# akankshabaranwal/graph-algorithm-image-segmentation-GPGPU

Hardware: NVIDIA B200
Metric: Mpixel/s end-to-end segmentation (1080p, Boruvka-Felzenszwalb, 4-connected) (higher is better)
Workload: dtype f32+u64

## Files before the change

graph-algorithm-image-segmentation-gpgpu_b200/__init__.py:

```python
import ctypes as C
import os
import subprocess

import numpy as np

_HERE = os.path.dirname(os.path.abspath(__file__))
_ROOT = os.path.dirname(_HERE)
CSRC = os.path.join(_HERE, "csrc")
LIB_PATH = os.environ.get("GSEG_LIB") or os.path.join(_HERE, "libgseg.so")
CLI_PATH = os.path.join(_HERE, "gseg")
BATCH_PATH = os.path.join(_HERE, "gseg_batch")
HEADER = os.path.join(_ROOT, "include", "gseg.h")

FELZ, HIER, SUPERPIX = 0, 1, 2
MEM_HOST, MEM_DEVICE = 0, 1
FLAG_HOST_LOOP = 1
FLAG_NO_DEDUP = 2
CAP_SUPERPIX, CAP_WIDE_SIGMA, CAP_LEVELS, CAP_JPEG = 1, 2, 4, 8
JPEG_AUTO, JPEG_OWN, JPEG_NVJPEG = 0, 1, 2
OUT_NONE, OUT_LABELS, OUT_HIERARCHY = 0, 1, 2
POOL_MAXLEVELS = 64

NVCC_FLAGS = ["-gencode", "arch=compute_100a,code=sm_100a", "-O3", "-lineinfo", "-std=c++17",
              "-Xcompiler", "-fPIC,-ffp-contract=off"]
# ... 88 lines not shown
    L.gseg_segment_jpeg_async.argtypes = [vp, vp, C.c_size_t, C.POINTER(Params), C.POINTER(i32), C.POINTER(i32)]
    L.gseg_input_rgb.argtypes = [vp, vp, i32]
    L.gseg_jpeg_decode_async.argtypes = [vp, vp, C.c_size_t, vp, C.c_size_t, vp, C.POINTER(i32), C.POINTER(i32)]
    L.gseg_set_jpeg_backend.argtypes = [vp, i32]
    L.gseg_jpeg_backend_used.argtypes = [vp]
    L.gseg_num_levels.argtypes = [vp]
    L.gseg_num_components.argtypes = [vp, i32]
    L.gseg_labels.argtypes = [vp, i32, vp, i32]
    L.gseg_labels_async.argtypes = [vp, i32, vp, i32]
    L.gseg_sync.argtypes = [vp]
    L.gseg_labels_all.argtypes = [vp, vp, i32, i32]
    L.gseg_colorize.argtypes = [vp, i32, u64, vp, i32]
    L.gseg_weights.argtypes = [vp, vp, i32]
    L.gseg_blurred.argtypes = [vp, vp, i32]
    L.gseg_stats.argtypes = [vp, C.POINTER(RoundStat), i32]
    i64 = C.c_int64
    L.gseg_export_graph.argtypes = [vp, i32, C.POINTER(i64), C.POINTER(i64), vp, vp, vp, vp, vp, i64, i64]
    L.gseg_blurred_rows.argtypes = [vp, i32, i32, vp, i32]
    L.gseg_segment_graph.argtypes = [vp, i64, vp, vp, i64, vp, vp, vp, C.POINTER(Params), vp]
    L.gseg_synth.argtypes = [vp, vp, i32, i32, u64, i32]
    L.gseg_synth_rows.argtypes = [vp, vp, i32, i32, i32, u64, i32]
    L.gseg_set_profiling.argtypes = [vp, i32]
    L.gseg_profile_read.argtypes = [vp, C.POINTER(KernelTime), i32]
    L.gseg_launch_count.argtypes = [vp]
    L.gseg_launch_count.restype = C.c_longlong
    L.gseg_sort_pairs_u64.argtypes = [vp, vp, vp, C.c_int64, i32, i32]
    L.gseg_reserve.argtypes = [vp, C.c_uint32]
    L.gseg_set_dedup.argtypes = [vp, i32, C.c_uint32, C.c_uint32, C.c_uint32]
    L.gseg_host_alloc.argtypes = [C.c_size_t]
    L.gseg_host_alloc.restype = vp
# ... 295 lines not shown
        Int = np.ascontiguousarray(Int, np.float32)
        ea = np.ascontiguousarray(ea, np.uint32)
        eb = np.ascontiguousarray(eb, np.uint32)
        w = np.ascontiguousarray(w, np.float32)
        out = np.empty(len(size), np.int32)
        n = self._ck(self.L.gseg_segment_graph(self.h, len(size), size.ctypes.data, Int.ctypes.data, len(ea),
                                               ea.ctypes.data, eb.ctypes.data, w.ctypes.data, C.byref(p),
                                               out.ctypes.data), "gseg_segment_graph")
        return out, n

    def stats(self):
        arr = (RoundStat * 64)()
        n = self._ck(self.L.gseg_stats(self.h, arr, 64), "gseg_stats")
        return [(arr[i].n_components, arr[i].n_edges, arr[i].n_merged, arr[i].phase) for i in range(n)]

    def dedup_rounds(self):
        arr = (RoundStat * 64)()
        n = self._ck(self.L.gseg_stats(self.h, arr, 64), "gseg_stats")
        return [(i, arr[i].n_edges, arr[i].n_edges_dedup) for i in range(n) if arr[i].n_edges_dedup]

    def timeline(self):
        arr = (RoundStat * 64)()
        n = self._ck(self.L.gseg_stats(self.h, arr, 64), "gseg_stats")
        return [(i, arr[i].in_tail, arr[i].us_end, arr[i].us_S, arr[i].us_R, arr[i].us_E, arr[i].n_pages) for i in range(n)]

    def set_profiling(self, on):
        self._ck(self.L.gseg_set_profiling(self.h, int(on)), "gseg_set_profiling")

    def profile(self):
        arr = (KernelTime * 1024)()
# ... 29 lines not shown
```

graph-algorithm-image-segmentation-gpgpu_b200/csrc/gseg_api.cu:

```cuda
#include <cuda_runtime.h>
#include <dlfcn.h>
#include <nvjpeg.h>
#include <limits.h>
#include <stddef.h>
#include <math.h>
#include <stdio.h>
#include <stdlib.h>
#include <string.h>

#include <new>
#include <vector>

#include "../../include/gseg.h"
#include "gseg_kernels.cuh"
#include "gseg_sort.cuh"
#include "gseg_dedup.cuh"
#include "gseg_jpeg.hpp"
#include "gseg_jpeg.cuh"

#define GSEG_MAXMARK 1024
#define GRID_CAP (148 * 8)

struct GsegHead {
    GsegRunParams p;
    RoundState st;
    u32 Vnext, error, ticketC, ticketE, doneE, Eacc[GSEG_MAXR + 1];
    u32 map_skip[GSEG_MAXR + 1], resume_phase;
    u32 stDedupIn[GSEG_MAXR + 1], stDedupOut[GSEG_MAXR + 1];
};
static_assert(offsetof(GsegCtl, Eacc) == offsetof(GsegHead, Eacc), "GsegHead must mirror the head of GsegCtl");
static_assert(offsetof(GsegCtl, resume_phase) == offsetof(GsegHead, resume_phase), "GsegHead must mirror the head of GsegCtl");
static_assert(offsetof(GsegCtl, stDedupOut) == offsetof(GsegHead, stDedupOut), "GsegHead must mirror the head of GsegCtl");
#define GSEG_EPOCHS_PER_RUN (2u * GSEG_MAXR + 8u + 32u)

#define R0_STAGE_MAX_PPW 128

static const size_t TAIL_SMEM = (2 * (size_t)GSEG_TAIL_STAGE + 2 * (NTT / 32)) * sizeof(u32);

struct gseg_ctx {
    int device, max_w, max_h;
    size_t Vmax;
    int Dmax;
    cudaStream_t stream, own_stream;
    uint8_t *d_rgb;
    float *d_tmp, *d_planes, *d_G, *d_wgrid;
    u32 *d_wsel, *d_succ, *d_rank;
    u64 *d_best[2];
    uint2 *d_attr[2];
    long long *d_csum[2];
    float4 *d_cmean[2];
    uint2 *d_eab[2];
    u32 *d_ew[2], *d_pcnt[2], *d_poff[2], *d_pscan;
    u32 *d_arena;
    size_t arena_cap;
    u64 *d_statusC, *d_statusE;
    size_t ntilesC, ntilesE;
    int *d_labels[2];
    GsegCtl *d_ctl, *h_ctl;
    GsegHead *h_head;
    int num_sms, occ_mult;
    u32 filter_shift;
    u32 r0_stage_ppw;
    int tail_cluster;
    bool tail_cluster_env;
    u32 tail_E, tail_V, tail_P;
    u32 run_tail_E, run_tail_V;
    int nbig_hint;
    int hint_w, hint_h, hint_variant, hint_conn;
    SortScratch sort;
    DedupDev *d_dd;
    u64 *d_winner;
    size_t dd_cap;
    u32 dd_min_edges, dd_min_ratio, dd_V;
    bool dd_on;
    bool dd_skip;
    u64 *d_xkeys;
    u32 *d_xvals, *d_xkeep, *d_xw, *x_w;
// ... 188 lines not shown
        cudaFuncSetAttribute(k_tail<false>, cudaFuncAttributeMaxDynamicSharedMemorySize, (int)TAIL_SMEM);
        if (const char *ev = getenv("GSEG_TAIL_CLUSTER")) want = atoi(ev);
        ctx->tail_cluster = fit_tail_cluster(want);
        ctx->tail_cluster_env = getenv("GSEG_TAIL_CLUSTER") != nullptr;
        ctx->tail_E = 256u * 1024u; ctx->tail_V = 64u * 1024u; ctx->tail_P = 4096u;
        if (const char *ev = getenv("GSEG_TAIL_P")) ctx->tail_P = (u32)strtoul(ev, nullptr, 10);
        if (const char *ev = getenv("GSEG_TAIL_E")) ctx->tail_E = (u32)strtoul(ev, nullptr, 10);
        if (const char *ev = getenv("GSEG_TAIL_V")) ctx->tail_V = (u32)strtoul(ev, nullptr, 10);
        ctx->nbig_hint = -1;
        ctx->occ_mult = 4;
        if (const char *ev = getenv("GSEG_OCC_MULT")) ctx->occ_mult = atoi(ev) > 0 ? atoi(ev) : 4;
        ctx->filter_shift = 6;
        if (const char *ev = getenv("GSEG_FILTER_SHIFT")) ctx->filter_shift = (u32)atoi(ev);
        ctx->r0_stage_ppw = R0_STAGE_MAX_PPW;
        if (const char *ev = getenv("GSEG_R0_STAGE_PPW")) ctx->r0_stage_ppw = (u32)strtoul(ev, nullptr, 10);
    }
    if (e != cudaSuccess) {
        fprintf(stderr, "gseg_create: %s\n", cudaGetErrorString(e));
        gseg_destroy(ctx);
        return GSEG_E_CUDA;
    }
    memset(ctx->h_ctl, 0, sizeof(GsegCtl));
    *out = ctx;
    return GSEG_OK;
}


struct NvJpegApi {
    void *lib;
    decltype(&nvjpegCreateSimple) create;
// ... 385 lines not shown
static void launch_r0_edges(gseg_ctx *c, cudaStream_t s, size_t V, const GsegBufs &B) {
    static bool attr[64] = {false};
    if (!attr[c->device & 63]) { cudaFuncSetAttribute(k_r0_edges<D, SP, true>, cudaFuncAttributeMaxDynamicSharedMemorySize, (int)R0_SMEM); attr[c->device & 63] = true; }
    const size_t pages = (size_t)D * ((V + GSEG_PAGE - 1) / GSEG_PAGE);
    const size_t ntiles = (pages + NT / 32 - 1) / (NT / 32);
    const int grid = (int)(ntiles < (size_t)c->num_sms * c->occ_mult ? ntiles : (size_t)c->num_sms * c->occ_mult);
    if (pages <= (size_t)c->r0_stage_ppw * grid * (NT / 32)) {
        mark(c, s, "k_r0_edges", 0);
        k_r0_edges<D, SP, true><<<grid, NT, R0_SMEM, s>>>(c->d_ctl, B);
    } else {
        mark(c, s, "k_r0_edges_rl", 0);
        k_r0_edges<D, SP, false><<<grid, NT, 0, s>>>(c->d_ctl, B);
    }
}

static void enqueue_round0(gseg_ctx *c, cudaStream_t s) {
    const size_t V = (size_t)c->w * c->h;
    const int variant = c->params.variant, D = c->D;
    const bool sp = variant == GSEG_SUPERPIX;
    const GsegBufs B = bufs_of(c);
    const int ntiles = ((c->w + TW - 1) / TW) * ((c->h + TH - 1) / TH);
    const int ntilesG = ((c->w + TW - 1) / TW) * ((c->h + GH - 1) / GH);
    const int R = c->h_head->p.mask_len - 1;
    if (R >= 1 && R <= 8) {
        mark(c, s, "k_blur_tile", 0);
        switch (R) {
        case 1: launch_blur<1>(c, s, ntiles); break;
        case 2: launch_blur<2>(c, s, ntiles); break;
        case 3: launch_blur<3>(c, s, ntiles); break;
        case 4: launch_blur<4>(c, s, ntiles); break;
// ... 33 lines not shown
    const int cap = c->num_sms * c->occ_mult;
    if (Pb > GSEG_PSCAN_INLINE) {
        mark(c, s, "k_page_scan", r);
        k_page_scan<<<grid_for(Pb, 1024, 64), 1024, 0, s>>>(c->d_ctl, B);
    }
    mark(c, s, "k_succ_scan", r);
    if (sp) k_succ_scan<true><<<grid_for(Vb, NT * CPT, cap) + 1, NT, 0, s>>>(c->d_ctl, B);
    else k_succ_scan<false><<<grid_for(Vb, NT * CPT, cap) + 1, NT, 0, s>>>(c->d_ctl, B);
    mark(c, s, "k_relabel", r);
    if (sp) k_relabel<false, true><<<grid_for(Vb, NT, cap), NT, 0, s>>>(c->d_ctl, B);
    else k_relabel<false, false><<<grid_for(Vb, NT, cap), NT, 0, s>>>(c->d_ctl, B);
    if (sp) {
        mark(c, s, "k_means", r);
        k_means<<<grid_for(Vb, NT, cap), NT, 0, s>>>(c->d_ctl, B);
    }
    mark(c, s, "k_edges", r);
    if (sp) k_edges<true><<<grid_for(Pb, NT / 32, cap), NT, 0, s>>>(c->d_ctl, B);
    else k_edges<false><<<grid_for(Pb, NT / 32, cap), NT, 0, s>>>(c->d_ctl, B);
}

static u32 dedup_V(const gseg_ctx *c) {
    const u32 v = c->dd_V > 2u ? c->dd_V : 2u;
    return v < 65536u ? v : 65536u;
}
static bool dedup_enabled(const gseg_ctx *c) {
    return c->dd_on && c->params.variant != GSEG_SUPERPIX && !(c->params.flags & GSEG_FLAG_NO_DEDUP);
}
static bool dedup_enqueue(const gseg_ctx *c) {
    return dedup_enabled(c) &&
           !(c->dd_skip && c->hint_w == c->w && c->hint_h == c->h && c->hint_variant == c->params.variant && c->hint_conn == c->params.connectivity);
}
static void enqueue_dedup(gseg_ctx *c, cudaStream_t s, int round) {
    const GsegBufs B = bufs_of(c);
// ... 242 lines not shown
    hp->max_levels = p->max_levels > 0 ? p->max_levels : INT_MAX;
    hp->arena_cap = (u32)ctx->arena_cap; hp->edge_slots = (u32)edge_slots(ctx);
    hp->epoch_base = ctx->epoch_next;
    hp->mask_len = len;
    hp->filter_shift = ctx->filter_shift;
    hp->tail_E = ctx->run_tail_E = host_loop ? 0u : ctx->tail_E;
    hp->tail_V = ctx->run_tail_V = host_loop ? 0u : ctx->tail_V;
    hp->tail_P = ctx->tail_P;
    hp->no_dedup = dedup_enabled(ctx) ? 0u : 1u; hp->dd_V = dedup_V(ctx);
    ctx->epoch_next += GSEG_EPOCHS_PER_RUN;
    hh->st.V = (u32)((size_t)w * h); hh->st.E = 0; hh->st.round = 0; hh->st.phase = PH_PRED; hh->st.levels = 0; hh->st.map_off = 0; hh->st.P = 0; hh->st.pad = 0;
    hh->Vnext = hh->st.V; hh->error = DERR_NONE; hh->ticketC = 0; hh->ticketE = 0; hh->doneE = 0;
    memset(hh->Eacc, 0, sizeof(hh->Eacc));
    memset(hh->map_skip, 0, sizeof(hh->map_skip)); hh->resume_phase = PH_DONE;
    memset(hh->stDedupIn, 0, sizeof(hh->stDedupIn)); memset(hh->stDedupOut, 0, sizeof(hh->stDedupOut));
    CK(cudaMemcpyAsync(ctx->d_ctl, hh, sizeof(GsegHead), cudaMemcpyHostToDevice, ctx->stream));

    ctx->n_marks = 0;
    enqueue_round0(ctx, ctx->stream);
    CK(cudaGetLastError());
    if (!host_loop) {
        int nbig = ctx->nbig_hint;
        if (nbig < 0 || ctx->hint_w != w || ctx->hint_h != h || ctx->hint_variant != p->variant ||
            ctx->hint_conn != p->connectivity)
            nbig = estimate_nbig(ctx);
        if (nbig > R - 1) nbig = R - 1;
        const size_t V = (size_t)w * h;
        for (int r = 1; r <= nbig; ++r) enqueue_round(ctx, ctx->stream, r, V, (size_t)ctx->D * (V / GSEG_PAGE + 1));
        if (dedup_enqueue(ctx)) enqueue_dedup(ctx, ctx->stream, -1);
        CK(cudaGetLastError());
// ... 377 lines not shown
    hp->epoch_base = ctx->epoch_next;
    hp->filter_shift = ctx->filter_shift;
    const bool host_loop = (p->flags & GSEG_FLAG_HOST_LOOP) != 0;
    hp->tail_E = ctx->run_tail_E = host_loop ? 0u : ctx->tail_E;
    hp->tail_V = ctx->run_tail_V = host_loop ? 0u : ctx->tail_V;
    hp->tail_P = ctx->tail_P;
    hp->no_dedup = dedup_enabled(ctx) ? 0u : 1u; hp->dd_V = dedup_V(ctx);
    ctx->epoch_next += GSEG_EPOCHS_PER_RUN;
    const u32 P = (u32)((E + GSEG_PAGE - 1) / GSEG_PAGE);
    hh->st.V = (u32)V; hh->st.E = (u32)E; hh->st.round = 1; hh->st.phase = PH_PRED; hh->st.levels = 0; hh->st.map_off = 0;
    hh->st.P = P; hh->st.pad = 0;
    hh->Vnext = (u32)V; hh->error = DERR_NONE; hh->ticketC = 0; hh->ticketE = 0; hh->doneE = 0;
    memset(hh->Eacc, 0, sizeof(hh->Eacc));
    memset(hh->map_skip, 0, sizeof(hh->map_skip)); hh->resume_phase = PH_DONE;
    memset(hh->stDedupIn, 0, sizeof(hh->stDedupIn)); memset(hh->stDedupOut, 0, sizeof(hh->stDedupOut));
    CK(cudaMemcpyAsync(ctx->d_ctl, hh, sizeof(GsegHead), cudaMemcpyHostToDevice, s));
    ctx->n_marks = 0;
    const GsegBufs B = bufs_of(ctx);
    if (P) { ++ctx->launches; k_graph_init<<<grid_for(P, NT / 32), NT, 0, s>>>(B, (u32)E, P); }
    CK(cudaGetLastError());
    ctx->nbig_hint = -1;
    int rc;
    if (host_loop) {
        rc = readback(ctx);
        for (int go; !rc && (go = run_continues(ctx)) != 0;) {
            if (go < 0) { rc = go; break; }
            if (dedup_wanted_host(ctx)) {
                enqueue_dedup(ctx, s, (int)ctx->h_ctl->st.round);
                CK(cudaGetLastError());
                if ((rc = readback(ctx)) != 0) break;
// ... 166 lines not shown
        out[i].n_edges = i == 0 ? 0 : (hc->stDedupIn[i] ? hc->stDedupIn[i] : hc->stE[i]);
        out[i].n_merged = hc->stM[i];
        out[i].phase = (int32_t)hc->stP[i];
        const bool tail = hc->stTail[i] != 0;
        out[i].in_tail = tail ? 1 : 0;
        out[i].n_pages = (int32_t)hc->stPages[i];
        out[i].n_edges_dedup = deduped ? (int32_t)(hc->stDedupOut[i] ? hc->stDedupOut[i] : hc->stE[i]) : 0;
        out[i].us_end = (float)((double)(hc->t_end[i] - hc->t_start) * 1e-3);
        out[i].us_S = tail ? (float)((double)(hc->t_S[i] - hc->t_begin[i]) * 1e-3) : 0.f;
        out[i].us_R = tail ? (float)((double)(hc->t_R[i] - hc->t_S[i]) * 1e-3) : 0.f;
        out[i].us_E = tail ? (float)((double)(hc->t_end[i] - hc->t_R[i]) * 1e-3) : 0.f;
    }
    return n;
}

extern "C" int gseg_synth_rows(gseg_ctx *ctx, uint8_t *out, int w, int y_first, int nrows, uint64_t seed, int mem_kind) {
    if (!ctx || !out || w < 1 || nrows < 1 || y_first < 0) return GSEG_E_ARG;
    if (mem_kind != GSEG_MEM_HOST && mem_kind != GSEG_MEM_DEVICE) return GSEG_E_ARG;
    if (mem_kind == GSEG_MEM_HOST && (size_t)w * nrows > ctx->Vmax) return GSEG_E_SIZE;
    if (ctx->pending) return GSEG_E_STATE;
    CK(cudaSetDevice(ctx->device));
    const size_t V = (size_t)w * nrows;
    uint8_t *dst = mem_kind == GSEG_MEM_DEVICE ? out : ctx->d_rgb;
    ++ctx->launches;
    k_synth<<<grid_for(V, NT), NT, 0, ctx->stream>>>(dst, w, nrows, seed, y_first);
    CK(cudaGetLastError());
    if (mem_kind != GSEG_MEM_DEVICE) CK(cudaMemcpyAsync(out, dst, 3 * V, cudaMemcpyDeviceToHost, ctx->stream));
    CK(cudaStreamSynchronize(ctx->stream));
    return GSEG_OK;
}
// ... 33 lines not shown
    const double En = (r + 1 < (int)h->st.round) ? h->stE[r + 1] : h->st.E;
    const bool sp = c->params.variant == GSEG_SUPERPIX;
    const double acc = sp ? 40 : 16;
    double a = 0, s = 0;
    if (!strcmp(name, "k_blur_tile") || !strcmp(name, "k_blur_h")) a = s = 3 * V0 + 12 * V0;
    else if (!strcmp(name, "k_blur_v")) a = s = 12 * V0 + 12 * V0;
    else if (!strcmp(name, "k_sobel")) a = s = 12 * V0 + 4 * V0;
    else if (!strcmp(name, "k_r0_graph")) a = s = (sp ? 16 : 12) * V0 + 4 * E0 + 8 * V0 + (4 + acc) * Vn;
    else if (!strcmp(name, "k_relabel")) {
        const double attr_in = r == 0 ? (sp ? 12 * V : 0) : (sp ? 32 : 8) * V, out = (sp ? 32 : 8) * Vn;
        a = 4 * V + 4 * V + 4 * V + 4 * V + attr_in + 4 * (V - Vn) + out;
        s = 4 * V + 4 * Vn + 4 * V + attr_in + 4 * (V - Vn) + out;
    }
    else if (!strcmp(name, "k_r0_edges") || !strcmp(name, "k_r0_edges_rl")) { a = 4 * E0 + 8 * E0 + 12 * En + 8 * Vn; s = 4 * E0 + 4 * V0 + 12 * En + 8 * Vn; }
    else if (!strcmp(name, "k_succ_scan")) { a = 8 * V + 8 * V + 16 * V + 8 * V + 8 * V + (4 + acc) * Vn; s = 8 * V + 8 * V + 8 * V + 8 * V + (4 + acc) * Vn; }
    else if (!strcmp(name, "k_edges")) { a = 12 * E + 8 * E + 12 * En + 8 * Vn + (sp ? 32 * En : 0); s = 12 * E + 4 * V + 12 * En + 8 * Vn + (sp ? 16 * Vn : 0); }
    else if (!strcmp(name, "k_means")) a = s = 32 * Vn + 16 * Vn;
    else if (!strcmp(name, "k_page_scan")) a = s = 8.0 * h->stPages[r];
    *algo = a; *strict = s;
}

extern "C" int gseg_profile_read(gseg_ctx *ctx, gseg_kernel_time *out, int cap) {
    if (!ctx || !ctx->valid) return GSEG_E_STATE;
    CK(cudaSetDevice(ctx->device));
    CK(cudaStreamSynchronize(ctx->stream));
    int n = 0;
    for (int i = 0; i + 1 < ctx->n_marks && n < cap; ++i) {
        if (!ctx->mark_name[i]) continue;
        float ms = 0.f;
        if (cudaEventElapsedTime(&ms, ctx->ev[i], ctx->ev[i + 1]) != cudaSuccess) { cudaGetLastError(); continue; }
        if (out) {
// ... 10 lines not shown
```

graph-algorithm-image-segmentation-gpgpu_b200/csrc/gseg_device.cuh:

```cuda
#pragma once
#include <cuda_runtime.h>
#include <stdint.h>

typedef unsigned int u32;
typedef unsigned long long u64;

#define GSEG_KEY_NONE 0xFFFFFFFFFFFFFFFFull
#define GSEG_INF_BITS 0x7F800000u
#define GSEG_MAXR 64
#define GSEG_MAXMASK 64
#define GSEG_PAGE 256u

enum { PH_PRED = 0, PH_MINSIZE = 1, PH_DONE = 2 };
enum { DERR_NONE = 0, DERR_SCAN = 1, DERR_ARENA = 2, DERR_CHASE = 3, DERR_JPEG = 4 , DERR_CHECK = 100  };

#ifdef GSEG_CHECKED
#define GSEG_CHK(ctl, cond, site)                                                         \
    do {                                                                                  \
        if (!(cond)) atomicMax(&(const_cast<GsegCtl *>(ctl))->error, (u32)DERR_CHECK + (u32)(site)); \
    } while (0)
#else
#define GSEG_CHK(ctl, cond, site) ((void)0)
#endif

// ... 21 lines not shown
    u32 P;
    u32 pad;
};

struct GsegCtl {
    GsegRunParams p;
    RoundState st;
    u32 Vnext;
    u32 error;
    u32 ticketC, ticketE;
    u32 doneE;
    u32 Eacc[GSEG_MAXR + 1];
    u32 map_skip[GSEG_MAXR + 1];
    u32 resume_phase;
    u32 stDedupIn[GSEG_MAXR + 1], stDedupOut[GSEG_MAXR + 1];
    u32 map_off[GSEG_MAXR + 1];
    u32 stV[GSEG_MAXR], stE[GSEG_MAXR], stM[GSEG_MAXR], stP[GSEG_MAXR], stVafter[GSEG_MAXR];
    u32 stTail[GSEG_MAXR], stPages[GSEG_MAXR];
    u64 t_start, t_end[GSEG_MAXR], t_begin[GSEG_MAXR], t_S[GSEG_MAXR], t_R[GSEG_MAXR];
};

struct GsegBufs {
    float *planes, *G, *wgrid;
    u32 *succ, *rank, *wsel, *arena;
    u64 *best[2];
    uint2 *attr[2];
    long long *csum[2];
    float4 *cmean[2];
    uint2 *eab[2];
    u32 *ew[2];
// ... 240 lines not shown
```

graph-algorithm-image-segmentation-gpgpu_b200/csrc/gseg_kernels.cuh:

```cuda
#pragma once
#include <cooperative_groups.h>

#include "gseg_device.cuh"

namespace cg = cooperative_groups;

#define NT 256
#ifndef GSEG_LB_SUCC
#define GSEG_LB_SUCC 4
#endif
#ifndef GSEG_LB_EDGES
#define GSEG_LB_EDGES 4
#endif
#define NTT 1024
#define CPT 4
#ifndef RUNWIN
#define RUNWIN 4
#endif

#define TW 64
#ifndef TH
#define TH 32
#endif
#define BW (TW + 4)
// ... 873 lines not shown
    const u32 nwarp = blockDim.x >> 5, nw = gridDim.x * nwarp;
    const bool staged = SPREAD && stage != nullptr && st.V <= GSEG_TAIL_STAGE;
    u32 *s_map = stage, *s_bhi = stage + GSEG_TAIL_STAGE;
    if (staged) {
        for (u32 i = threadIdx.x; i < st.V; i += blockDim.x) s_map[i] = __ldcg(map + i);
        if (filter) {
            const u32 *bhi = reinterpret_cast<const u32 *>(B.best[nxt]) + 1;
            for (u32 i = threadIdx.x; i < Vnext; i += blockDim.x) s_bhi[i] = ld_relaxed_u32(bhi + 2 * (size_t)i);
        }
        __syncthreads();
    }
    constexpr int NQ = ROWS / RW;
    const u32 wid = threadIdx.x >> 5, q = SPREAD ? (wid & (NQ - 1)) : 0u, grp = wid / NQ;
    u32 *s_ex = stage + 2 * GSEG_TAIL_STAGE;
    u32 esum = 0, parity = 0;
    for (u32 g = SPREAD ? grp * gridDim.x + blockIdx.x : blockIdx.x * nwarp + wid; g < ngroups; g += SPREAD ? gridDim.x * (nwarp / NQ) : nw) {
        u32 mycnt = 0u, myoff = 0u;
        if ((u32)lane < G && G * g + lane < P) { mycnt = __ldcg(pc + G * g + lane); myoff = __ldcg(po + G * g + lane); }
        const u32 incl = warp_incl_scan(mycnt, lane);
        const u32 excl = incl - mycnt, cnt = __shfl_sync(0xFFFFFFFFu, incl, 31);
        const u32 out_base = G > 1u ? __ldcg(B.pscan + G * g) : __shfl_sync(0xFFFFFFFFu, myoff, 0);
        u32 written = 0;
        for (u32 c0 = 0; c0 < cnt; c0 += GSEG_PAGE) {
            u32 a[RW], b[RW], wv[RW], m[RW];
#pragma unroll
            for (int j = 0; j < RW; ++j) {
                const u32 i = c0 + 32u * (q * RW + j) + lane;
                u32 k = 0u;
                if (G > 1u) {
#pragma unroll
                    for (u32 step = 8u; step; step >>= 1) {
                        const u32 e = __shfl_sync(0xFFFFFFFFu, excl, (int)(k + step));
                        if (k + step < G && e <= i) k += step;
                    }
                }
                const u32 src = __shfl_sync(0xFFFFFFFFu, myoff, (int)k) + (i - __shfl_sync(0xFFFFFFFFu, excl, (int)k));
                uint2 ab = make_uint2(0u, 0u);
                wv[j] = 0u;
                if (i < cnt) {
                    GSEG_CHK(ctl, src < ctl->p.edge_slots, 7);
                    ab = __ldcg(eab + src); wv[j] = __ldcg(ew + src);
                    GSEG_CHK(ctl, ab.x < st.V && ab.y < st.V, 8);
                }
                a[j] = ab.x; b[j] = ab.y;
            }
            u32 sub = 0;
#pragma unroll
            for (int j = 0; j < RW; ++j) {
                bool keep = false;
                if (c0 + 32u * (q * RW + j) + lane < cnt) {
                    if (staged) { a[j] = s_map[a[j]]; b[j] = s_map[b[j]]; }
                    else { a[j] = ld_prev<!SPREAD>(map + a[j]); b[j] = ld_prev<!SPREAD>(map + b[j]); }
                    keep = a[j] != b[j];
                }
                m[j] = __ballot_sync(0xFFFFFFFFu, keep);
                sub += __popc(m[j]);
// ... 47 lines not shown
        if (q == 0u) {
            if (lane == 0) { B.pcnt[nxt][g] = written; B.poff[nxt][g] = out_base; }
            esum += written;
        }
    }
    if (lane == 0 && esum) atomicAdd(&ctl->Eacc[st.round], esum);
}
template <bool SP, bool SPREAD = false>
__device__ __forceinline__ void phase_E(GsegCtl *ctl, const GsegBufs &B, const RoundState &st, u32 Vnext, u32 *stage = nullptr) {
    if (SPREAD) {
        const u32 G = group_size(st), ngroups = (st.P + G - 1u) / G;
        if (ngroups <= 2u * gridDim.x * (blockDim.x >> 5)) phase_E_rows<SP, true, 2>(ctl, B, st, Vnext, stage);
        else phase_E_rows<SP, true, GSEG_PAGE / 32>(ctl, B, st, Vnext, stage);
    } else {
        phase_E_rows<SP, false, GSEG_PAGE / 32>(ctl, B, st, Vnext, stage);
    }
}

__device__ __forceinline__ void phase_M(const GsegBufs &B, int nxt, u32 Vnext) {
    for (u32 n = ((threadIdx.x >> 5) * gridDim.x + blockIdx.x) * 32u + (threadIdx.x & 31u); n < Vnext; n += gridDim.x * blockDim.x)
        B.cmean[nxt][n] = mean_of(B.csum[nxt], B.attr[nxt], n);
}

template <bool R0, bool SP>
__global__ void __launch_bounds__(NT) k_relabel(const GsegCtl *ctl, GsegBufs B) {
    const RoundState st = ctl->st;
    if (st.phase == PH_DONE || in_tail(ctl, st)) return;
    phase_R<NT, R0, SP>(ctl, B, st);
}
__global__ void __launch_bounds__(NT) k_means(const GsegCtl *ctl, GsegBufs B) {
// ... 23 lines not shown
        if (i < P) B.pscan[i] = wpre + inc - v;
        __syncthreads();
    }
}
template <bool SP>
__global__ void __launch_bounds__(NT, GSEG_LB_SUCC) k_succ_scan(GsegCtl *ctl, GsegBufs B) {
    __shared__ u32 sh[66];
    const RoundState st = ctl->st;
    if (st.phase == PH_DONE || in_tail(ctl, st)) return;
    if (blockIdx.x == gridDim.x - 1) {
        if (group_size(st) > 1u && st.P <= GSEG_PSCAN_INLINE) block_scan_pages(B.pcnt[st.round & 1], st.P, B.pscan, sh);
        return;
    }
    phase_S<SP, false>(ctl, B, st, sh);
}
template <bool SP>
__global__ void __launch_bounds__(NT, GSEG_LB_EDGES) k_edges(GsegCtl *ctl, GsegBufs B) {
    const RoundState st = ctl->st;
    if (st.phase == PH_DONE || in_tail(ctl, st)) return;
    phase_E<SP>(ctl, B, st, ctl->Vnext);
    last_block_advance(ctl, st, group_size(st));
}

template <bool SP>
__global__ void __launch_bounds__(NTT, 1) k_tail(GsegCtl *ctl, GsegBufs B) {
    extern __shared__ __align__(16) u32 tail_stage[];
    __shared__ u32 sh[66];
    cg::cluster_group cl = cg::this_cluster();
    const bool writer = blockIdx.x == 0 && threadIdx.x == 0;
    RoundState st = load_state(ctl);
    cl.sync();
    while (st.phase != PH_DONE && in_tail(ctl, st)) {
        if (writer) ctl->t_begin[st.round] = globaltimer_ns();
        const u32 G = group_size(st);
        if (G > 1u && blockIdx.x == gridDim.x - 1) block_scan_pages(B.pcnt[st.round & 1], st.P, B.pscan, sh);
// ... 267 lines not shown
```

include/gseg.h:

```cpp
#ifndef GSEG_H
#define GSEG_H

#include <stddef.h>
#include <stdint.h>

#ifdef __cplusplus
extern "C" {
#endif

#define GSEG_VERSION 200

#define GSEG_FELZ 0
#define GSEG_HIER 1
#define GSEG_SUPERPIX 2

#define GSEG_MEM_HOST 0
#define GSEG_MEM_DEVICE 1

#define GSEG_FLAG_HOST_LOOP 1u

#define GSEG_FLAG_NO_DEDUP 2u

typedef enum gseg_status {
    GSEG_OK = 0,
// ... 108 lines not shown
                      int64_t *n_joined_edges);

#define GSEG_JPEG_AUTO 0
#define GSEG_JPEG_OWN 1
#define GSEG_JPEG_NVJPEG 2
int gseg_jpeg_info(const void *jpeg, size_t nbytes, int *w, int *h);
int gseg_segment_jpeg_async(gseg_ctx *ctx, const void *jpeg, size_t nbytes, const gseg_params *params, int *w, int *h);
int gseg_segment_jpeg(gseg_ctx *ctx, const void *jpeg, size_t nbytes, const gseg_params *params, int *w, int *h);
int gseg_input_rgb(gseg_ctx *ctx, uint8_t *out_rgb, int mem_kind);
int gseg_jpeg_decode_async(gseg_ctx *ctx, const void *jpeg, size_t nbytes, uint8_t *rgb_out_device, size_t out_capacity,
                           void *cuda_stream, int *w, int *h);
int gseg_set_jpeg_backend(gseg_ctx *ctx, int backend);
int gseg_jpeg_backend_used(const gseg_ctx *ctx);

int gseg_stats(const gseg_ctx *ctx, gseg_round_stat *out, int cap);

int gseg_synth(gseg_ctx *ctx, uint8_t *out_rgb, int w, int h, uint64_t seed, int mem_kind);
int gseg_synth_rows(gseg_ctx *ctx, uint8_t *out_rgb, int w, int y_first, int nrows, uint64_t seed, int mem_kind);

typedef struct gseg_kernel_time {
    char name[24];
    int32_t round;
    float ms;
    double algo_bytes;
    double strict_bytes;
} gseg_kernel_time;
int gseg_set_profiling(gseg_ctx *ctx, int on);
int gseg_profile_read(gseg_ctx *ctx, gseg_kernel_time *out, int cap);
long long gseg_launch_count(const gseg_ctx *ctx);
long long gseg_compaction_count(const gseg_ctx *ctx);
// ... 43 lines not shown
```

Measured before the change: 10050.

## Prefetch edge-group metadata and pages in edge compaction; add optional bulk-copy staged variant

In the default edge-compaction path, each warp now loads group count and offset metadata two groups ahead. It also issues L1 prefetches for the upcoming group's edge and weight cache lines, and switches those loads from L2-only to L1-cached. A new staged kernel variant, selected by an environment threshold that defaults to off, double-buffers whole edge groups into shared memory with bulk async copies and mbarriers. It also records per-round group statistics. The goal is to hide global-memory latency on the edge gather, at the cost of extra registers and an extra L1 prefetch instruction stream.

After: 9452 (median of 6 runs). -5.9%, worse.

```diff
diff --git a/graph-algorithm-image-segmentation-gpgpu_b200/__init__.py b/graph-algorithm-image-segmentation-gpgpu_b200/__init__.py
--- a/graph-algorithm-image-segmentation-gpgpu_b200/__init__.py
+++ b/graph-algorithm-image-segmentation-gpgpu_b200/__init__.py
@@ -126,6 +126,7 @@
     L.gseg_weights.argtypes = [vp, vp, i32]
     L.gseg_blurred.argtypes = [vp, vp, i32]
     L.gseg_stats.argtypes = [vp, C.POINTER(RoundStat), i32]
+    L.gseg_edge_groups.argtypes = [vp, C.POINTER(C.c_int32), i32]
     i64 = C.c_int64
     L.gseg_export_graph.argtypes = [vp, i32, C.POINTER(i64), C.POINTER(i64), vp, vp, vp, vp, vp, i64, i64]
     L.gseg_blurred_rows.argtypes = [vp, i32, i32, vp, i32]
@@ -451,6 +452,11 @@
         n = self._ck(self.L.gseg_stats(self.h, arr, 64), "gseg_stats")
         return [(arr[i].n_components, arr[i].n_edges, arr[i].n_merged, arr[i].phase) for i in range(n)]
 
+    def edge_groups(self):
+        arr = (C.c_int32 * (3 * 64))()
+        n = self._ck(self.L.gseg_edge_groups(self.h, arr, 64), "gseg_edge_groups")
+        return [(arr[3 * i], arr[3 * i + 1], arr[3 * i + 2]) for i in range(n)]
+
     def dedup_rounds(self):
         arr = (RoundStat * 64)()
         n = self._ck(self.L.gseg_stats(self.h, arr, 64), "gseg_stats")
diff --git a/graph-algorithm-image-segmentation-gpgpu_b200/csrc/gseg_api.cu b/graph-algorithm-image-segmentation-gpgpu_b200/csrc/gseg_api.cu
--- a/graph-algorithm-image-segmentation-gpgpu_b200/csrc/gseg_api.cu
+++ b/graph-algorithm-image-segmentation-gpgpu_b200/csrc/gseg_api.cu
@@ -27,13 +27,16 @@
     u32 Vnext, error, ticketC, ticketE, doneE, Eacc[GSEG_MAXR + 1];
     u32 map_skip[GSEG_MAXR + 1], resume_phase;
     u32 stDedupIn[GSEG_MAXR + 1], stDedupOut[GSEG_MAXR + 1];
+    u32 stGroups[GSEG_MAXR + 1][3];
 };
 static_assert(offsetof(GsegCtl, Eacc) == offsetof(GsegHead, Eacc), "GsegHead must mirror the head of GsegCtl");
 static_assert(offsetof(GsegCtl, resume_phase) == offsetof(GsegHead, resume_phase), "GsegHead must mirror the head of GsegCtl");
 static_assert(offsetof(GsegCtl, stDedupOut) == offsetof(GsegHead, stDedupOut), "GsegHead must mirror the head of GsegCtl");
+static_assert(offsetof(GsegCtl, stGroups) == offsetof(GsegHead, stGroups), "GsegHead must mirror the head of GsegCtl");
 #define GSEG_EPOCHS_PER_RUN (2u * GSEG_MAXR + 8u + 32u)
 
 #define R0_STAGE_MAX_PPW 128
+#define EDGE_STAGE_MAX_PPW 0
 
 static const size_t TAIL_SMEM = (2 * (size_t)GSEG_TAIL_STAGE + 2 * (NTT / 32)) * sizeof(u32);
 
@@ -61,6 +64,7 @@
     int num_sms, occ_mult;
     u32 filter_shift;
     u32 r0_stage_ppw;
+    u32 edge_stage_ppw;
     int tail_cluster;
     bool tail_cluster_env;
     u32 tail_E, tail_V, tail_P;
@@ -279,6 +283,8 @@
         if (const char *ev = getenv("GSEG_FILTER_SHIFT")) ctx->filter_shift = (u32)atoi(ev);
         ctx->r0_stage_ppw = R0_STAGE_MAX_PPW;
         if (const char *ev = getenv("GSEG_R0_STAGE_PPW")) ctx->r0_stage_ppw = (u32)strtoul(ev, nullptr, 10);
+        ctx->edge_stage_ppw = EDGE_STAGE_MAX_PPW;
+        if (const char *ev = getenv("GSEG_EDGE_STAGE_PPW")) ctx->edge_stage_ppw = (u32)strtoul(ev, nullptr, 10);
     }
     if (e != cudaSuccess) {
         fprintf(stderr, "gseg_create: %s\n", cudaGetErrorString(e));
@@ -694,6 +700,20 @@
     }
 }
 
+template <bool SP>
+static void launch_edges(gseg_ctx *c, cudaStream_t s, int r, size_t Pb, int cap, const GsegBufs &B) {
+    static bool attr[64] = {false};
+    if (!attr[c->device & 63]) { cudaFuncSetAttribute(k_edges<SP, true>, cudaFuncAttributeMaxDynamicSharedMemorySize, (int)E_SMEM); attr[c->device & 63] = true; }
+    const int grid = grid_for(Pb, NT / 32, cap);
+    if (Pb <= (size_t)c->edge_stage_ppw * grid * (NT / 32)) {
+        mark(c, s, "k_edges", r);
+        k_edges<SP, true><<<grid, NT, E_SMEM, s>>>(c->d_ctl, B);
+    } else {
+        mark(c, s, "k_edges_rl", r);
+        k_edges<SP, false><<<grid, NT, 0, s>>>(c->d_ctl, B);
+    }
+}
+
 static void enqueue_round0(gseg_ctx *c, cudaStream_t s) {
     const size_t V = (size_t)c->w * c->h;
     const int variant = c->params.variant, D = c->D;
@@ -757,9 +777,8 @@
         mark(c, s, "k_means", r);
         k_means<<<grid_for(Vb, NT, cap), NT, 0, s>>>(c->d_ctl, B);
     }
-    mark(c, s, "k_edges", r);
-    if (sp) k_edges<true><<<grid_for(Pb, NT / 32, cap), NT, 0, s>>>(c->d_ctl, B);
-    else k_edges<false><<<grid_for(Pb, NT / 32, cap), NT, 0, s>>>(c->d_ctl, B);
+    if (sp) launch_edges<true>(c, s, r, Pb, cap, B);
+    else launch_edges<false>(c, s, r, Pb, cap, B);
 }
 
 static u32 dedup_V(const gseg_ctx *c) {
@@ -1032,6 +1051,7 @@
     memset(hh->Eacc, 0, sizeof(hh->Eacc));
     memset(hh->map_skip, 0, sizeof(hh->map_skip)); hh->resume_phase = PH_DONE;
     memset(hh->stDedupIn, 0, sizeof(hh->stDedupIn)); memset(hh->stDedupOut, 0, sizeof(hh->stDedupOut));
+    memset(hh->stGroups, 0, sizeof(hh->stGroups));
     CK(cudaMemcpyAsync(ctx->d_ctl, hh, sizeof(GsegHead), cudaMemcpyHostToDevice, ctx->stream));
 
     ctx->n_marks = 0;
@@ -1439,6 +1459,7 @@
     memset(hh->Eacc, 0, sizeof(hh->Eacc));
     memset(hh->map_skip, 0, sizeof(hh->map_skip)); hh->resume_phase = PH_DONE;
     memset(hh->stDedupIn, 0, sizeof(hh->stDedupIn)); memset(hh->stDedupOut, 0, sizeof(hh->stDedupOut));
+    memset(hh->stGroups, 0, sizeof(hh->stGroups));
     CK(cudaMemcpyAsync(ctx->d_ctl, hh, sizeof(GsegHead), cudaMemcpyHostToDevice, s));
     ctx->n_marks = 0;
     const GsegBufs B = bufs_of(ctx);
@@ -1635,6 +1656,17 @@
     return n;
 }
 
+extern "C" int gseg_edge_groups(const gseg_ctx *ctx, int32_t *out, int cap) {
+    if (!ctx || !ctx->valid) return GSEG_E_STATE;
+    const GsegCtl *hc = ctx->h_ctl;
+    const int n = (int)hc->st.round;
+    for (int i = 0; i < n && i < cap && out; ++i) {
+        for (int j = 0; j < 3; ++j) out[3 * i + j] = (int32_t)hc->stGroups[i][j];
+        out[3 * i] -= out[3 * i + 1] + out[3 * i + 2];
+    }
+    return n;
+}
+
 extern "C" int gseg_synth_rows(gseg_ctx *ctx, uint8_t *out, int w, int y_first, int nrows, uint64_t seed, int mem_kind) {
     if (!ctx || !out || w < 1 || nrows < 1 || y_first < 0) return GSEG_E_ARG;
     if (mem_kind != GSEG_MEM_HOST && mem_kind != GSEG_MEM_DEVICE) return GSEG_E_ARG;
@@ -1698,7 +1730,7 @@
     }
     else if (!strcmp(name, "k_r0_edges") || !strcmp(name, "k_r0_edges_rl")) { a = 4 * E0 + 8 * E0 + 12 * En + 8 * Vn; s = 4 * E0 + 4 * V0 + 12 * En + 8 * Vn; }
     else if (!strcmp(name, "k_succ_scan")) { a = 8 * V + 8 * V + 16 * V + 8 * V + 8 * V + (4 + acc) * Vn; s = 8 * V + 8 * V + 8 * V + 8 * V + (4 + acc) * Vn; }
-    else if (!strcmp(name, "k_edges")) { a = 12 * E + 8 * E + 12 * En + 8 * Vn + (sp ? 32 * En : 0); s = 12 * E + 4 * V + 12 * En + 8 * Vn + (sp ? 16 * Vn : 0); }
+    else if (!strcmp(name, "k_edges") || !strcmp(name, "k_edges_rl")) { a = 12 * E + 8 * E + 12 * En + 8 * Vn + (sp ? 32 * En : 0); s = 12 * E + 4 * V + 12 * En + 8 * Vn + (sp ? 16 * Vn : 0); }
     else if (!strcmp(name, "k_means")) a = s = 32 * Vn + 16 * Vn;
     else if (!strcmp(name, "k_page_scan")) a = s = 8.0 * h->stPages[r];
     *algo = a; *strict = s;
diff --git a/graph-algorithm-image-segmentation-gpgpu_b200/csrc/gseg_device.cuh b/graph-algorithm-image-segmentation-gpgpu_b200/csrc/gseg_device.cuh
--- a/graph-algorithm-image-segmentation-gpgpu_b200/csrc/gseg_device.cuh
+++ b/graph-algorithm-image-segmentation-gpgpu_b200/csrc/gseg_device.cuh
@@ -59,6 +59,7 @@
     u32 map_skip[GSEG_MAXR + 1];
     u32 resume_phase;
     u32 stDedupIn[GSEG_MAXR + 1], stDedupOut[GSEG_MAXR + 1];
+    u32 stGroups[GSEG_MAXR + 1][3];
     u32 map_off[GSEG_MAXR + 1];
     u32 stV[GSEG_MAXR], stE[GSEG_MAXR], stM[GSEG_MAXR], stP[GSEG_MAXR], stVafter[GSEG_MAXR];
     u32 stTail[GSEG_MAXR], stPages[GSEG_MAXR];
diff --git a/graph-algorithm-image-segmentation-gpgpu_b200/csrc/gseg_kernels.cuh b/graph-algorithm-image-segmentation-gpgpu_b200/csrc/gseg_kernels.cuh
--- a/graph-algorithm-image-segmentation-gpgpu_b200/csrc/gseg_kernels.cuh
+++ b/graph-algorithm-image-segmentation-gpgpu_b200/csrc/gseg_kernels.cuh
@@ -911,12 +911,33 @@
     const u32 wid = threadIdx.x >> 5, q = SPREAD ? (wid & (NQ - 1)) : 0u, grp = wid / NQ;
     u32 *s_ex = stage + 2 * GSEG_TAIL_STAGE;
     u32 esum = 0, parity = 0;
+    auto meta = [&](u32 gg, u32 &cnt, u32 &off) {
+        cnt = 0u; off = 0u;
+        if ((u32)lane < G && G * gg + lane < P) { cnt = __ldcg(pc + G * gg + lane); off = __ldcg(po + G * gg + lane); }
+        if (lane == 31 && G > 1u && gg < ngroups) off = __ldcg(B.pscan + G * gg);
+    };
+    u32 n1c = 0u, n1o = 0u, n2c = 0u, n2o = 0u;
+    if constexpr (!SPREAD) { meta(blockIdx.x * nwarp + wid, n1c, n1o); meta(blockIdx.x * nwarp + wid + nw, n2c, n2o); }
     for (u32 g = SPREAD ? grp * gridDim.x + blockIdx.x : blockIdx.x * nwarp + wid; g < ngroups; g += SPREAD ? gridDim.x * (nwarp / NQ) : nw) {
         u32 mycnt = 0u, myoff = 0u;
-        if ((u32)lane < G && G * g + lane < P) { mycnt = __ldcg(pc + G * g + lane); myoff = __ldcg(po + G * g + lane); }
+        if constexpr (SPREAD) {
+            if ((u32)lane < G && G * g + lane < P) { mycnt = __ldcg(pc + G * g + lane); myoff = __ldcg(po + G * g + lane); }
+        } else {
+            mycnt = n1c; myoff = n1o; n1c = n2c; n1o = n2o;
+            meta(g + 2u * nw, n2c, n2o);
+            const u32 lo = __shfl_sync(0xFFFFFFFFu, n1o, 0), hi = __shfl_sync(0xFFFFFFFFu, n1o + n1c, (int)G - 1);
+            if (hi > lo && hi - lo <= 4u * GSEG_PAGE) {
+                const char *pab = reinterpret_cast<const char *>(eab), *pw = reinterpret_cast<const char *>(ew);
+                const size_t la = (8 * (size_t)lo) >> 7, na = ((8 * (size_t)hi - 1) >> 7) - la + 1;
+                const size_t lw = (4 * (size_t)lo) >> 7, nwl = ((4 * (size_t)hi - 1) >> 7) - lw + 1;
+                for (u32 l = lane; l < na; l += 32u) asm volatile("prefetch.global.L1 [%0];" ::"l"(pab + ((la + l) << 7)));
+                for (u32 l = lane; l < nwl; l += 32u) asm volatile("prefetch.global.L1 [%0];" ::"l"(pw + ((lw + l) << 7)));
+            }
+        }
         const u32 incl = warp_incl_scan(mycnt, lane);
         const u32 excl = incl - mycnt, cnt = __shfl_sync(0xFFFFFFFFu, incl, 31);
-        const u32 out_base = G > 1u ? __ldcg(B.pscan + G * g) : __shfl_sync(0xFFFFFFFFu, myoff, 0);
+        const u32 out_base = !SPREAD ? __shfl_sync(0xFFFFFFFFu, myoff, G > 1u ? 31 : 0)
+                             : G > 1u ? __ldcg(B.pscan + G * g) : __shfl_sync(0xFFFFFFFFu, myoff, 0);
         u32 written = 0;
         for (u32 c0 = 0; c0 < cnt; c0 += GSEG_PAGE) {
             u32 a[RW], b[RW], wv[RW], m[RW];
@@ -936,7 +957,8 @@
                 wv[j] = 0u;
                 if (i < cnt) {
                     GSEG_CHK(ctl, src < ctl->p.edge_slots, 7);
-                    ab = __ldcg(eab + src); wv[j] = __ldcg(ew + src);
+                    if (SPREAD) { ab = __ldcg(eab + src); wv[j] = __ldcg(ew + src); }
+                    else { ab = __ldca(eab + src); wv[j] = __ldca(ew + src); }
                     GSEG_CHK(ctl, ab.x < st.V && ab.y < st.V, 8);
                 }
                 a[j] = ab.x; b[j] = ab.y;
@@ -1014,6 +1036,190 @@
         else phase_E_rows<SP, true, GSEG_PAGE / 32>(ctl, B, st, Vnext, stage);
     } else {
         phase_E_rows<SP, false, GSEG_PAGE / 32>(ctl, B, st, Vnext, stage);
+    }
+}
+
+#define E_RUNS 8
+#define E_CAP_AB (GSEG_PAGE + 2 * E_RUNS)
+#define E_CAP_W (GSEG_PAGE + 6 * E_RUNS)
+#define E_BUF (2 * E_CAP_AB + E_CAP_W)
+#define E_SMEM ((NT / 32) * (2 * E_BUF * 4 + 16))
+__device__ __forceinline__ u32 e_run_word(u32 cnt, u32 off) {
+    if (cnt == 0u) return 0u;
+    const u32 end = off + cnt;
+    return min(cnt, GSEG_PAGE + 1u) | ((off & 1u) + (end & 1u)) << 16 | ((off & 3u) + ((4u - (end & 3u)) & 3u)) << 24;
+}
+__device__ __forceinline__ bool e_fits(u32 tot) {
+    const u32 n = tot & 0xFFFFu;
+    return n != 0u && n <= GSEG_PAGE && n + ((tot >> 16) & 0xFFu) <= E_CAP_AB && n + (tot >> 24) <= E_CAP_W;
+}
+template <bool SP>
+__device__ __forceinline__ void phase_E_pages(GsegCtl *ctl, const GsegBufs &B, const RoundState &st, u32 Vnext, u32 *smem) {
+    constexpr int ROWS = GSEG_PAGE / 32;
+    const int lane = threadIdx.x & 31;
+    const u32 lt = (1u << lane) - 1u, wid = threadIdx.x >> 5;
+    const int cur = st.round & 1, nxt = cur ^ 1;
+    const u32 E = st.E, P = st.P;
+    const uint2 *eab = B.eab[cur];
+    const u32 *ew = B.ew[cur];
+    const u32 *pc = B.pcnt[cur], *po = B.poff[cur];
+    const u32 *map = B.arena + st.map_off;
+    const bool filter = (E >> ctl->p.filter_shift) > Vnext;
+    const u32 G = group_size(st), ngroups = (P + G - 1u) / G;
+    if (blockIdx.x == 0 && threadIdx.x == 0) ctl->ticketC = 0;
+    const u32 nw = gridDim.x * (NT / 32);
+    u64 *bar = reinterpret_cast<u64 *>(smem) + 2 * wid;
+    u32 *buf = smem + 4 * (NT / 32) + wid * 2 * E_BUF;
+    auto meta = [&](u32 g, u32 &cnt, u32 &off) {
+        cnt = 0u; off = 0u;
+        if ((u32)lane < G && G * g + lane < P) { cnt = __ldcg(pc + G * g + lane); off = __ldcg(po + G * g + lane); }
+        if (lane == 31 && G > 1u && g < ngroups) off = __ldcg(B.pscan + G * g);
+    };
+    auto plan = [&](u32 cnt, u32 off) {
+        const u32 x = e_run_word(cnt, off);
+        return warp_incl_scan(x, lane) - x;
+    };
+    auto issue = [&](u32 cnt, u32 off, u32 ex, u32 tot, u32 k) {
+        const u32 n = tot & 0xFFFFu;
+        if (lane == 0) mbar_expect_tx(bar + k, 8u * (n + ((tot >> 16) & 0xFFu)) + 4u * (n + (tot >> 24)));
+        __syncwarp();
+        if (cnt) {
+            const u32 sab = (ex & 0xFFFFu) + ((ex >> 16) & 0xFFu), sw = (ex & 0xFFFFu) + (ex >> 24), end = off + cnt;
+            u32 *dst = buf + k * E_BUF;
+            fence_proxy_async();
+            bulk_copy(dst + 2 * sab, eab + (off & ~1u), 8u * (((end + 1u) & ~1u) - (off & ~1u)), bar + k);
+            bulk_copy(dst + 2 * E_CAP_AB + sw, ew + (off & ~3u), 4u * (((end + 3u) & ~3u) - (off & ~3u)), bar + k);
+        }
+    };
+    u32 g = blockIdx.x * (NT / 32) + wid;
+    u32 c_cnt, c_off, c_ex, n_cnt, n_off;
+    meta(g, c_cnt, c_off);
+    c_ex = plan(c_cnt, c_off);
+    if (lane == 0) { mbar_init(bar); mbar_init(bar + 1); }
+    __syncwarp();
+    {
+        const u32 tot = __shfl_sync(0xFFFFFFFFu, c_ex, 31);
+        if (g < ngroups && e_fits(tot)) issue(c_cnt, c_off, c_ex, tot, 0u);
+    }
+    meta(g + nw, n_cnt, n_off);
+    u32 esum = 0, kp = 0;
+    for (; g < ngroups; g += nw, kp ^= 4u) {
+        const u32 k = kp >> 2;
+        const u32 n_ex = plan(n_cnt, n_off), n_tot = __shfl_sync(0xFFFFFFFFu, n_ex, 31);
+        __syncwarp();
+        if (g + nw < ngroups && e_fits(n_tot)) issue(n_cnt, n_off, n_ex, n_tot, k ^ 1u);
+        const u32 mycnt = c_cnt, myoff = c_off, ex = c_ex, tot = __shfl_sync(0xFFFFFFFFu, c_ex, 31);
+        const u32 out_base = __shfl_sync(0xFFFFFFFFu, myoff, G > 1u ? 31 : 0);
+        c_cnt = n_cnt; c_off = n_off; c_ex = n_ex;
+        meta(g + 2u * nw, n_cnt, n_off);
+        const bool staged = e_fits(tot);
+        u32 excl = ex & 0xFFFFu, cnt = tot & 0xFFFFu;
+        if (!staged && cnt) {
+            const u32 incl = warp_incl_scan(mycnt, lane);
+            excl = incl - mycnt;
+            cnt = __shfl_sync(0xFFFFFFFFu, incl, 31);
+        }
+        const u32 dab = (ex & 0xFFFFu) + ((ex >> 16) & 0xFFu) + (myoff & 1u) - excl;
+        const u32 dw = (ex & 0xFFFFu) + (ex >> 24) + (myoff & 3u) - excl;
+        const u32 dsrc = myoff - excl;
+        uint2 *s_ab = reinterpret_cast<uint2 *>(buf + k * E_BUF);
+        u32 *s_w = buf + k * E_BUF + 2 * E_CAP_AB;
+        if (staged) { mbar_wait(bar + k, (kp >> k) & 1u); kp ^= 1u << k; }
+        else if (lane == 0) atomicAdd(&ctl->stGroups[st.round][cnt ? 1 : 2], 1u);
+        u32 written = 0;
+        for (u32 c0 = 0; c0 < cnt; c0 += GSEG_PAGE) {
+#pragma unroll
+            for (int j = 0; j < ROWS; ++j) {
+                const u32 i = c0 + 32u * j + lane;
+                u32 r = 0u;
+                if (G > 1u) {
+#pragma unroll
+                    for (u32 step = 8u; step; step >>= 1) {
+                        const u32 e = __shfl_sync(0xFFFFFFFFu, excl, (int)(r + step));
+                        if (r + step < G && e <= i) r += step;
+                    }
+                }
+                const u32 sa = __shfl_sync(0xFFFFFFFFu, staged ? dab : dsrc, (int)r) + i;
+                const u32 sw = __shfl_sync(0xFFFFFFFFu, dw, (int)r) + i;
+                uint2 ab = make_uint2(0u, 0u);
+                u32 wv = 0u;
+                if (i < cnt) {
+                    if (staged) { ab = s_ab[sa]; wv = s_w[sw]; }
+                    else {
+                        GSEG_CHK(ctl, sa < ctl->p.edge_slots, 7);
+                        ab = __ldcg(eab + sa); wv = __ldcg(ew + sa);
+                    }
+                    GSEG_CHK(ctl, ab.x < st.V && ab.y < st.V, 8);
+                }
+                if (staged) __syncwarp();
+                s_ab[32 * j + lane] = ab; s_w[32 * j + lane] = wv;
+            }
+            u32 mrow = 0u, total = 0u;
+            {
+                u32 a[ROWS], b[ROWS];
+#pragma unroll
+                for (int j = 0; j < ROWS; ++j) {
+                    a[j] = b[j] = 0u;
+                    if (c0 + 32u * j + lane < cnt) {
+                        const uint2 ab = s_ab[32 * j + lane];
+                        a[j] = ld_prev<true>(map + ab.x); b[j] = ld_prev<true>(map + ab.y);
+                    }
+                }
+#pragma unroll
+                for (int j = 0; j < ROWS; ++j) {
+                    const bool in = c0 + 32u * j + lane < cnt;
+                    const u32 m = __ballot_sync(0xFFFFFFFFu, in && a[j] != b[j]);
+                    if (lane == j) mrow = m;
+                    total += __popc(m);
+                    if (in) s_ab[32 * j + lane] = make_uint2(a[j], b[j]);
+                }
+            }
+            u32 rowoff = out_base + written;
+            GSEG_CHK(ctl, (unsigned long long)out_base + written + total <= ctl->p.edge_slots, 9);
+            if (filter) {
+                const u32 *bhi = reinterpret_cast<const u32 *>(B.best[nxt]) + 1;
+#pragma unroll
+                for (int h = 0; h < ROWS; h += ROWS / 2) {
+                    u32 fa[ROWS / 2], fb[ROWS / 2];
+#pragma unroll
+                    for (int j = 0; j < ROWS / 2; ++j) {
+                        fa[j] = fb[j] = 0xFFFFFFFFu;
+                        if ((__shfl_sync(0xFFFFFFFFu, mrow, h + j) >> lane) & 1u) {
+                            const uint2 ab = s_ab[32 * (h + j) + lane];
+                            fa[j] = ld_relaxed_u32(bhi + 2 * (size_t)ab.x); fb[j] = ld_relaxed_u32(bhi + 2 * (size_t)ab.y);
+                        }
+                    }
+#pragma unroll
+                    for (int j = 0; j < ROWS / 2; ++j) {
+                        const u32 m = __shfl_sync(0xFFFFFFFFu, mrow, h + j);
+                        if (m == 0u) continue;
+                        const bool act = (m >> lane) & 1u;
+                        const uint2 ab = s_ab[32 * (h + j) + lane];
+                        emit_row<SP, true>(B, nxt, rowoff + __popc(m & lt), act, ab.x, ab.y, s_w[32 * (h + j) + lane], fa[j], fb[j]);
+                        rowoff += __popc(m);
+                    }
+                }
+            } else {
+#pragma unroll
+                for (int j = 0; j < ROWS; ++j) {
+                    const u32 m = __shfl_sync(0xFFFFFFFFu, mrow, j);
+                    if (m == 0u) continue;
+                    const bool act = (m >> lane) & 1u;
+                    const uint2 ab = s_ab[32 * j + lane];
+                    emit_row<SP, false>(B, nxt, rowoff + __popc(m & lt), act, ab.x, ab.y, s_w[32 * j + lane]);
+                    rowoff += __popc(m);
+                }
+            }
+            written += total;
+            __syncwarp();
+        }
+        if (lane == 0) { B.pcnt[nxt][g] = written; B.poff[nxt][g] = out_base; }
+        esum += written;
+    }
+    if (lane == 0) {
+        if (esum) atomicAdd(&ctl->Eacc[st.round], esum);
+        const u32 g0 = blockIdx.x * (NT / 32) + wid;
+        if (g0 < ngroups) atomicAdd(&ctl->stGroups[st.round][0], (ngroups - 1u - g0) / nw + 1u);
     }
 }
 
@@ -1067,11 +1273,13 @@
     }
     phase_S<SP, false>(ctl, B, st, sh);
 }
-template <bool SP>
+template <bool SP, bool STAGED>
 __global__ void __launch_bounds__(NT, GSEG_LB_EDGES) k_edges(GsegCtl *ctl, GsegBufs B) {
+    extern __shared__ __align__(16) u32 e_stage[];
     const RoundState st = ctl->st;
     if (st.phase == PH_DONE || in_tail(ctl, st)) return;
-    phase_E<SP>(ctl, B, st, ctl->Vnext);
+    if constexpr (STAGED) phase_E_pages<SP>(ctl, B, st, ctl->Vnext, e_stage);
+    else phase_E<SP>(ctl, B, st, ctl->Vnext);
     last_block_advance(ctl, st, group_size(st));
 }
 
diff --git a/include/gseg.h b/include/gseg.h
--- a/include/gseg.h
+++ b/include/gseg.h
@@ -146,6 +146,7 @@
 int gseg_jpeg_backend_used(const gseg_ctx *ctx);
 
 int gseg_stats(const gseg_ctx *ctx, gseg_round_stat *out, int cap);
+int gseg_edge_groups(const gseg_ctx *ctx, int32_t *out, int cap);
 
 int gseg_synth(gseg_ctx *ctx, uint8_t *out_rgb, int w, int h, uint64_t seed, int mem_kind);
 int gseg_synth_rows(gseg_ctx *ctx, uint8_t *out_rgb, int w, int y_first, int nrows, uint64_t seed, int mem_kind);
```
